# tturturiello/lightweight-snappy

Hardware: AMD Instinct MI355X
Metric: compress + decompress MB/s at 1/2/4/8 MI355X; % HBM roofline; ratio vs ref (higher is better)
Workload: dtype u8

## Files before the change

### lightweight-snappy_amd/csrc/snappy_k2_emit.inc

```
    __shared__ __attribute__((aligned(16))) uint8_t stage_[kK2Stage + 4 + 4 * 64 + 16];
    auto *const stage = (__attribute__((address_space(3))) uint8_t *)stage_;
    const uint32_t lane = threadIdx.x;
    const uint32_t u = blockIdx.x;
    const uint32_t nt = ntok[u];
#if K2_RECORDS
    const uint64_t base = 0;
    const uint32_t L = rec.L;
#else
    const uint64_t base = (uint64_t)u * unit;
    const uint32_t L = (uint32_t)((n - base) < unit ? (n - base) : unit);
#endif
    const uint8_t *src = in + base;
    uint8_t *dst = out + offsets[u];
#if K2_RECORDS
    const uint32_t *tok = rec.tok, *tok_full = rec.tok_full;
#else
    const uint32_t *tok = reinterpret_cast<const uint32_t *>(tokens) + (uint64_t)u * tok_cap;
    const uint32_t *tok_full = reinterpret_cast<const uint32_t *>(tokens) + ((uint64_t)gridDim.x + u) * tok_cap;
#endif
    if (blockIdx.y == 0) {
        if (hdr_mode == SNAPPY_HDR_EVERY_UNIT) varint_put(L, dst, lane);
        else if (hdr_mode == SNAPPY_HDR_FIRST_UNIT && (K2_RECORDS || u == 0)) varint_put(header_value, dst, lane);
    }
    uint32_t kwn[kK2Per];
    auto load_kw = [&](uint32_t c, uint32_t *k) {
#pragma unroll
        for (uint32_t i = 0; i < kK2Per; i++) {
            const uint32_t t = c + kK2Per * lane + i;
            k[i] = tok[t < nt ? t : 0u];
        }
    };
    auto load_se = [&](uint32_t sg) {
#if K2_RECORDS
        return *reinterpret_cast<const uint2 *>(rec.segu + 2 * (sg * kK2Seg <= nt ? sg : 0u));
#else
        return *reinterpret_cast<const uint2 *>(seg_off + 2 * ((uint64_t)u * segs + (sg * kK2Seg <= nt ? sg : 0u)));
#endif
    };
    if (blockIdx.y * kK2Seg <= nt) load_kw(blockIdx.y * kK2Seg, kwn);
    uint2 sen = load_se(blockIdx.y);
    for (uint32_t sg = blockIdx.y; sg * kK2Seg <= nt; sg += gridDim.y) {
    const uint2 se = sen;
    sen = load_se(sg + gridDim.y);
    uint32_t o = se.x, carry = se.y;
    for (uint32_t c = sg * kK2Seg; c < (sg + 1) * kK2Seg && c <= nt; c += kK2Pass) {

    uint32_t gap[kK2Per], len[kK2Per], off[kK2Per], pe[kK2Per], litn[kK2Per], hl[kK2Per], sz[kK2Per];
    bool live[kK2Per];
    uint32_t lspan = 0;
    uint32_t kw[kK2Per];
#pragma unroll
    for (uint32_t i = 0; i < kK2Per; i++) kw[i] = kwn[i];
    {
        uint32_t cn = c + kK2Pass;
        if (!(cn < (sg + 1) * kK2Seg && cn <= nt)) cn = (sg + gridDim.y) * kK2Seg;
        if (cn <= nt) load_kw(cn, kwn);
    }
#pragma unroll
    for (uint32_t i = 0; i < kK2Per; i++) {
        const uint32_t t = c + kK2Per * lane + i;
        const bool has = t < nt;
        live[i] = t <= nt;
        const uint32_t k = has ? kw[i] : 0xFFFFFFFFu;
        const uint32_t lc = (k >> 16) & 0xFF, gc = k >> 24;
        off[i] = has ? k & 0xFFFF : 0u;
        gap[i] = has ? gc : 0u;
        len[i] = has ? lc + 4 : 0u;
        if (has && (lc == 255 || gc == 255)) {
            const uint32_t f = tok_full[t];
            gap[i] = f & 0xFFFF;
            len[i] = f >> 16;
        }
        lspan += gap[i] + len[i];
    }
    uint32_t span_tot;
    uint32_t cur = carry + wave_excl_scan(lspan, lane, &span_tot);
    uint32_t lsum = 0;
#pragma unroll
    for (uint32_t i = 0; i < kK2Per; i++) {
        const uint32_t t = c + kK2Per * lane + i;
        pe[i] = cur;
        litn[i] = t < nt ? gap[i] : (t == nt ? L - cur : 0u);
        cur += gap[i] + len[i];
        hl[i] = litn[i] ? (litn[i] <= 60 ? 1 : (litn[i] <= 256 ? 2 : 3)) : 0;
        sz[i] = hl[i] + litn[i] + ((live[i] && len[i]) ? copy_bytes(len[i], off[i]) : 0);
        lsum += sz[i];
    }
    uint32_t total;
    uint32_t rel = wave_excl_scan(lsum, lane, &total);
    const bool staged = total <= kK2Stage;
    const uint32_t sb = staged ? (uint32_t)(reinterpret_cast<uintptr_t>(dst + o) & 3) : 0u;
    uint64_t longs[kK2Per];
    uint32_t d0v[kK2Per];
    uint32_t lw[kK2Per][5], lsh[kK2Per];
    bool wide[kK2Per];
#pragma unroll
    for (uint32_t i = 0; i < kK2Per; i++) {
        wide[i] = base + pe[i] + 20 <= n;
        const bool ld = !SNAPPY_K2_NOLIT && staged && wide[i] && live[i] && litn[i] != 0 && litn[i] <= 16;
        const uintptr_t sa = reinterpret_cast<uintptr_t>(src + pe[i]);
        lsh[i] = (uint32_t)(sa & 3);
        const auto *aw = reinterpret_cast<const __attribute__((address_space(1))) uint32_t *>(
            ld ? sa - lsh[i] : reinterpret_cast<uintptr_t>(tok));
#pragma unroll
        for (uint32_t j = 0; j < 5; j++) lw[i][j] = aw[j];
    }
#pragma unroll
    for (uint32_t i = 0; i < kK2Per; i++) {
        const bool wide_ok = wide[i];
        if (staged) put_element_lds(stage, rel + sb, src, pe[i], litn[i], hl[i], len[i], off[i], wide_ok, live[i], lane,
                                    lw[i], lsh[i]);
        else if (live[i]) put_element(dst + o + rel, src, pe[i], litn[i], hl[i], len[i], off[i], wide_ok);
        longs[i] = __ballot(live[i] && litn[i] > 16);
        d0v[i] = rel + sb + hl[i];
        rel += sz[i];
    }
#pragma unroll
    for (uint32_t i = 0; i < kK2Per && !SNAPPY_K2_NOLIT; i++) {
        if (staged) k2_long_literals(stage, src, longs[i], litn[i], pe[i], d0v[i], lane);
        else k2_long_literals(dst + o, src, in + n, longs[i], litn[i], pe[i], d0v[i], lane);
    }
    if (staged) {
        __builtin_amdgcn_wave_barrier();
        uint8_t *g = dst + o;
        uint32_t head = (4 - sb) & 3;
        if (head > total) head = total;
        if (lane < head) g[lane] = stage[sb + lane];
        const uint32_t nw = (total - head) >> 2;
        uint32_t *gw = reinterpret_cast<uint32_t *>(g + head);
        const auto *sw = reinterpret_cast<const __attribute__((address_space(3))) uint32_t *>(stage + sb + head);
        for (uint32_t k = lane; k < nw; k += 64) gw[k] = sw[k];
        const uint32_t tail0 = head + 4 * nw;
        if (lane < total - tail0) g[tail0 + lane] = stage[sb + tail0 + lane];
    }
    __builtin_amdgcn_wave_barrier();
    o += total;
    carry += span_tot;
    }
    }
```

### lightweight-snappy_amd/csrc/snappy_kernels.hip

```cpp
#include <hip/hip_runtime.h>
#include <stdint.h>
#include <type_traits>

#include "snappy_kernels.h"

#ifndef SNAPPY_TU
#define SNAPPY_TU 0
#endif
#define SNAPPY_TU_COMPRESS (SNAPPY_TU != 2)
#define SNAPPY_TU_DECODE (SNAPPY_TU != 1)

#if ((defined(SNAPPY_K2_NOLIT) && SNAPPY_K2_NOLIT) || defined(SNAPPY_K4_NOFAR)) && !defined(SNAPPY_MEASUREMENT_BUILD)
#error "SNAPPY_K2_NOLIT / SNAPPY_K4_NOFAR write wrong output: measurement builds only (-DSNAPPY_MEASUREMENT_BUILD)"
#endif

namespace snappy_amd {

__device__ int amdgcn_writelane(int val, int lanesel, int old) __asm("llvm.amdgcn.writelane.i32");


constexpr uint32_t kTable = 4096;
constexpr uint32_t kMul = 0x1e35a7bdu;

typedef uint32_t u32x4 __attribute__((ext_vector_type(4)));
// ... 51 lines not shown
        if constexpr (BIG) _rv = REG_OF_V(_rr & (kRegs - 1));                                       \
        else _rv = REG_OF_V(_rr);                                                                   \
        _rv;                                                                                        \
    })

#define REG_PAIR_V(r, lo, hi)                                                                        \
    do {                                                                                             \
        asm volatile("s_set_gpr_idx_on %[ri], gpr_idx(SRC0)\n\tv_mov_b32 %[olo], v2\n\t"             \
                     "v_mov_b32 %[ohi], v3\n\ts_set_gpr_idx_off"                                     \
                     : [olo] "=&v"(lo), [ohi] "=&v"(hi)                                              \
                     : [ri] "s"((uint32_t)(r)), "{v[2:33]}"(g0), "{v[34:65]}"(g1), "{v[66:97]}"(g2),      \
                       "{v[98:129]}"(g3));                                                           \
    } while (0)
#define REG_PAIR(r, lo, hi)                                                                          \
    do {                                                                                             \
        const uint32_t _pr = (r);                                                                    \
        if constexpr (BIG) {                                  \
            const uint32_t _pq = _pr & (kRegs - 1);                                                  \
            if (__builtin_expect(_pq != kRegs - 1, 1)) REG_PAIR_V(_pq, lo, hi);                      \
            else { lo = REG_OF_V(kRegs - 1); hi = REG_OF_V(0); }                                     \
        } else {                                                                                     \
            REG_PAIR_V(_pr, lo, hi);                                                                 \
        }                                                                                            \
    } while (0)

#define DW_LANES(dd)                                                                                 \
    ({                                                                                               \
        const uint32_t _d = (dd);                                                                    \
        const uint32_t _R = _d >> 6, _l0 = _d & 63;                                                  \
                  \
                      \
        uint32_t _r0, _r1;                                                                           \
        REG_PAIR(_R, _r0, _r1);                                                                      \
        const uint32_t _m = lane >= _l0 ? _r0 : _r1;                                                 \
        (uint32_t)__builtin_amdgcn_ds_bpermute((int)((_d + lane) << 2), (int)_m);    \
    })

__device__ __forceinline__ uint32_t wave_shl1(uint32_t v)
{
    return (uint32_t)__builtin_amdgcn_update_dpp(0, (int)v, 0x130, 0xF, 0xF, true);
}
__device__ __forceinline__ uint32_t wave_shr1(uint32_t v)
{
    return (uint32_t)__builtin_amdgcn_update_dpp(0, (int)v, 0x138, 0xF, 0xF, true);
}

__device__ __forceinline__ uint32_t bytes_at(uint32_t cur, uint32_t next, uint32_t x)
{
    return __builtin_amdgcn_alignbyte(next, cur, x);
}

template <uint32_t D>
__device__ __forceinline__ uint32_t nearest_same_key(uint32_t w)
{
    static_assert(D <= 16, "d << 8 must stay below the key");
    const uint32_t x0 = w & 0xFFFF0000u;
    uint32_t xs = w, best = 0xFFFFFFFFu, k100;
    asm("v_mov_b32 %0, 0x100" : "=v"(k100));
#pragma unroll
    for (uint32_t d = 1; d <= D; d++) {
        xs = wave_shr1(xs) + k100;
        best = __builtin_elementwise_min(best, xs ^ x0);
    }
    return best;
}

__device__ __forceinline__ uint32_t varint_len(uint64_t v)
{
    uint32_t len = 1;
    while (v >= 128) { v >>= 7; len++; }
    return len;
}

__device__ __forceinline__ uint32_t literal_bytes(uint32_t n)
{
    return n + (n <= 60 ? 1 : (n <= 256 ? 2 : 3));
}

__device__ __forceinline__ uint32_t copy_bytes(uint32_t len, uint32_t off)
{
    const uint32_t n64 = len > 68 ? (len - 68 + 63) >> 6 : 0;
    const uint32_t rem = len - 64 * n64;
    const uint32_t has60 = rem > 64 ? 1u : 0u;
    const uint32_t last = has60 ? rem - 60 : rem;
    return 3 * (n64 + has60) + ((last < 12 && off < 2048) ? 2 : 3);
}

__device__ __forceinline__ uint32_t eqm(uint32_t x) { return (uint32_t)((int32_t)(x - 1) >> 31); }

template <int N>
__device__ __forceinline__ uint32_t shz(uint32_t v)
{
    return (uint32_t)__builtin_amdgcn_mov_dpp((int)v, 0x110 + N, 0xF, 0xF, true);
}

template <int N>
__device__ __forceinline__ uint32_t tconf_step(uint32_t h, uint32_t a, uint32_t notdup)
{
    const uint32_t hs = shz<N>(h), as = shz<N>(a);
    if constexpr (N == 1) return eqm(h ^ hs) | eqm(h ^ as) | (eqm(a ^ hs) & notdup);
    else return eqm(h ^ hs) | eqm(h ^ as) | eqm(a ^ hs);
}

template <int W>
__device__ __forceinline__ uint32_t tconf(uint32_t h, uint32_t a, uint32_t notdup)
{
    static_assert(W >= 1 && W <= 4, "W-probe rounds speculate at most 4 probes");
    uint32_t c = 0;
    if constexpr (W > 1) c |= tconf_step<1>(h, a, notdup);
    if constexpr (W > 2) c |= tconf_step<2>(h, a, notdup);
    if constexpr (W > 3) c |= tconf_step<3>(h, a, notdup);
    return c;
}

#ifndef SNAPPY_K1R_DMAX
#define SNAPPY_K1R_DMAX 13
#endif
#ifndef SNAPPY_K1R_DMAX64
#define SNAPPY_K1R_DMAX64 12
#endif
#ifndef SNAPPY_K1R_LSMIN
#define SNAPPY_K1R_LSMIN 4
#endif
#ifndef SNAPPY_K1R_RMIN
#define SNAPPY_K1R_RMIN 2
#endif
#ifndef SNAPPY_K1R_WINDOW
#define SNAPPY_K1R_WINDOW 4
#endif


#if defined(SNAPPY_K1R_LSTAMPS) || defined(SNAPPY_K1R_RSTAMPS)
#define MSTAMP(var)                                                                         \
    do {                                                                                    \
        __builtin_amdgcn_sched_barrier(0);                                                  \
        asm volatile("s_memtime %0\n\ts_waitcnt lgkmcnt(0)" : "=s"(var)::"memory");        \
        __builtin_amdgcn_sched_barrier(0);                                                  \
    } while (0)
#endif
#if defined(SNAPPY_K1R_RSTAMPS)
#define RSTAMP(var) MSTAMP(var)
#else
#define RSTAMP(var) do { } while (0)
#endif
#if defined(SNAPPY_K1R_LSTAMPS)
#define LSTAMP(var) MSTAMP(var)
#define LSEG(i, a, b) seg[i] += (b) - (a)
#else
#define LSTAMP(var) do { } while (0)
#define LSEG(i, a, b) do { } while (0)
#endif

#ifndef SNAPPY_K2_PASS
#define SNAPPY_K2_PASS 128u
#endif
constexpr uint32_t kK2Seg = SNAPPY_K2_SEG;
constexpr uint32_t kK2Pass = SNAPPY_K2_PASS;
[[maybe_unused]] constexpr uint32_t kK2Per = kK2Pass / 64;
static_assert(kK2Pass % 64 == 0 && kK2Seg % kK2Pass == 0, "K2: passes of 64 k tokens dividing a segment");

template <uint32_t CTRL, uint32_t ROWS>
__device__ __forceinline__ uint32_t dpp0(uint32_t x)
{
    return (uint32_t)__builtin_amdgcn_update_dpp(0, (int)x, CTRL, ROWS, 0xF, true);
}

__device__ __forceinline__ uint32_t wave_incl_scan(uint32_t x)
{
    x += dpp0<0x111, 0xF>(x);
    x += dpp0<0x112, 0xF>(x);
    x += dpp0<0x114, 0xF>(x);
    x += dpp0<0x118, 0xF>(x);
    x += dpp0<0x142, 0xA>(x);
    x += dpp0<0x143, 0xC>(x);
    return x;
}

__device__ __forceinline__ uint32_t wave_excl_scan(uint32_t v, uint32_t lane, uint32_t *total)
{
    (void)lane;
    const uint32_t x = wave_incl_scan(v);
    *total = (uint32_t)__builtin_amdgcn_readlane((int)x, 63);
    return x - v;
}


struct K1Record {
    uint32_t u;
    uint32_t L;
    const uint8_t *src;
    uint32_t *tok, *tok_full, *segu;
};

template <bool BIG, bool REC = false>
__device__ __forceinline__ void k1r_body(const uint8_t *__restrict__ in, uint64_t n, uint32_t unit,
                                         uint32_t hdr_mode, uint64_t header_value,
                                         uint2 *__restrict__ tokens, uint32_t tok_cap,
                                         uint32_t *__restrict__ ntok_out, uint32_t *__restrict__ sizes,
                                         uint32_t *__restrict__ seg_off, uint32_t segs, const K1Record rec = {})
{
    constexpr int W = SNAPPY_K1R_WINDOW;
    constexpr uint32_t DMAX = BIG ? SNAPPY_K1R_DMAX64 : SNAPPY_K1R_DMAX;
    static_assert(SNAPPY_K1R_LSMIN >= 4 && SNAPPY_K1R_LSMIN <= 32, "lane-space rounds need skip < 64 - 3");
    static_assert(DMAX >= 2 && DMAX <= 16, "DMAX: 2..16 (kcap <= 15 keeps the lane masks in range)");
    constexpr uint32_t kSlots = kTable + 1;
    constexpr uint32_t kTagBase = 2 * kSlots + 6;
    __shared__ __attribute__((aligned(16))) uint8_t tbl_[kTagBase + kSlots + 7];
    constexpr uint32_t kDummy = 2 * kTable;
    auto *const tbl = (__attribute__((address_space(3))) uint8_t *)tbl_;
#define TBL_READ3(adr)                                                                              \
    ({                                                                                             \
        const uint32_t _a = (adr);                                                                 \
        u16x2 _v;                                                                                  \
        _v.x = *(__attribute__((address_space(3))) uint16_t *)(tbl + _a);                          \
        _v.y = (uint16_t)tbl[(_a >> 1) + kTagBase];                                                \
        __builtin_bit_cast(uint32_t, _v);                                                          \
    })
#define TBL_WRITE3(adr, word)                                                                       \
    do {                                                                                           \
        const uint32_t _a = (adr), _w = (word);                                                    \
        *(__attribute__((address_space(3))) uint16_t *)(tbl + _a) = (uint16_t)_w;                   \
        tbl[(_a >> 1) + kTagBase] = (uint8_t)(_w >> 16);                                           \
    } while (0)
#define TBL_ADR(h) (2 * (h))
#define TBL_READ_ENT(adr)                                                                           \
    do {                                                                                           \
        const uint32_t _a = (adr);                                                                 \
        ent = *(__attribute__((address_space(3))) uint16_t *)(tbl + _a);                           \
        ent_t = tbl[(_a >> 1) + kTagBase];                                                         \
    } while (0)
#define TBL_READ(h) TBL_READ3(2 * (h))
#define TBL_WRITE(s, word) TBL_WRITE3(2 * (s), word)
#define TAG_OF(v) __builtin_amdgcn_ubfe((v) * kMul, shift - 8, 8)
#define TBL_INSERT(cond) TBL_WRITE3((cond) ? adr : kDummy, word)
#define LDS_ORDER() asm volatile("" ::: "memory")
#define TAG_EQ(e, w) ((((e) ^ (w)) & 0xFF0000u) == 0)
    const uint32_t lane = threadIdx.x;
    const uint32_t u = REC ? rec.u : blockIdx.x;
    const uint64_t base = REC ? 0 : (uint64_t)u * unit;
    const uint32_t L = REC ? rec.L : (uint32_t)((n - base) < unit ? (n - base) : unit);
    const uint8_t *src = REC ? rec.src : in + base;
#ifdef SNAPPY_K1R_STATS
    const uint64_t t_start = clock64();
    (void)t_start;
#endif

    v32 g0, g1, g2, g3;
    const bool aligned = ((reinterpret_cast<uintptr_t>(src) & 3) == 0);
    auto load_dw = [&](uint32_t k) -> uint32_t {
        const uint32_t b = 4 * k;
        uint32_t w = 0;
        if (b + 4 <= L && aligned) {
            w = __builtin_nontemporal_load(reinterpret_cast<const uint32_t *>(src + b));
        } else if (b < L) {
            for (uint32_t k = 0; k < 4; k++)
                if (b + k < L) w |= (uint32_t)src[b + k] << (8 * k);
        }
        return w;
    };
    auto load_word = [&](uint32_t i) -> uint32_t { return load_dw(64 * i + lane); };
#pragma unroll
    for (int i = 0; i < (int)kRegs; i++) {
        const uint32_t w = load_word(i);
        if (i < 32) g0[i] = w;
        else if (i < 64) g1[i - 32] = w;
        else if (i < 96) g2[i - 64] = w;
        else g3[i - 96] = w;
    }

    uint32_t seg_hi = kRegs;
#ifdef SNAPPY_K1R_STATS
    uint32_t n_farc = 0, n_reload = 0;
#define K1R_COUNT(x) (x)++
#else
#define K1R_COUNT(x) do { } while (0)
#endif
    __shared__ uint32_t ring_stage[64];
    uint32_t staged = 0;
    auto stage = [&](uint32_t sg) {
        if constexpr (BIG) {
            staged = 0;
            if (aligned && 256 * (sg + 1) <= L) {
                const uint32_t lds = (uint32_t)(uintptr_t)(__attribute__((address_space(3))) uint32_t *)ring_stage;
                uint32_t m0_save, voff;
                asm volatile("s_mov_b32 %0, m0\n\ts_mov_b32 m0, %2\n\tv_lshlrev_b32 %1, 2, %3\n\t"
                             "global_load_lds_dword %1, %4\n\ts_mov_b32 m0, %0"
                             : "=&s"(m0_save), "=&v"(voff)
                             : "s"(lds), "v"(lane), "s"(src + 256 * sg)
                             : "memory");
                staged = sg + 1;
            }
        }
    };
    stage(seg_hi);
    auto ring_to = [&](uint32_t need, auto pf) {
        if constexpr (BIG) {
            if (__builtin_expect(need <= seg_hi, 1)) return;
            uint32_t sg = need - seg_hi > kRegs ? need - kRegs : seg_hi;
            if (decltype(pf)::value && staged == sg + 1) {
                asm volatile("s_waitcnt vmcnt(0)" ::: "memory");
                const uint32_t lds = (uint32_t)(uintptr_t)(__attribute__((address_space(3))) uint32_t *)ring_stage;
                uint32_t w;
                asm volatile("v_lshl_add_u32 %0, %1, 2, %2\n\tds_read_b32 %0, %0\n\ts_waitcnt lgkmcnt(0)"
                             : "=&v"(w) : "v"(lane), "s"(lds) : "memory");
                REG_SET_V(sg & (kRegs - 1), w);
                sg++;
            }
// ... 938 lines not shown

template <bool BIG>
__device__ __forceinline__ void kr1_record(const uint8_t *__restrict__ in, const uint64_t *__restrict__ off_len,
                                           const uint32_t *__restrict__ list, const uint64_t *__restrict__ sbase,
                                           uint32_t *__restrict__ scratch, uint32_t *__restrict__ ntok_out,
                                           uint32_t *__restrict__ sizes)
{
    K1Record rec;
    rec.u = rfl(list[blockIdx.x]);
    rec.L = rfl((uint32_t)off_len[2 * (uint64_t)rec.u + 1]);
    rec.src = in + rfl64(off_len[2 * (uint64_t)rec.u]);
    const uint32_t tok_cap = records_tok_cap(rec.L);
    rec.tok = scratch + rfl64(sbase[rec.u]);
    rec.tok_full = rec.tok + tok_cap;
    rec.segu = rec.tok_full + tok_cap;
    k1r_body<BIG, true>(nullptr, 0, 0, SNAPPY_HDR_EVERY_UNIT, 0, nullptr, 0, ntok_out, sizes, nullptr, 0, rec);
}

#if SNAPPY_TU_COMPRESS
__global__ __launch_bounds__(64, 3) void kr1_match_records(const uint8_t *__restrict__ in,
                                                            const uint64_t *__restrict__ off_len,
                                                            const uint32_t *__restrict__ list,
                                                            const uint64_t *__restrict__ sbase,
                                                            uint32_t *__restrict__ scratch,
                                                            uint32_t *__restrict__ ntok_out,
                                                            uint32_t *__restrict__ sizes)
{
    kr1_record<false>(in, off_len, list, sbase, scratch, ntok_out, sizes);
}

__global__ __launch_bounds__(64, 3) void kr1_match_records64(const uint8_t *__restrict__ in,
                                                              const uint64_t *__restrict__ off_len,
                                                              const uint32_t *__restrict__ list,
                                                              const uint64_t *__restrict__ sbase,
                                                              uint32_t *__restrict__ scratch,
                                                              uint32_t *__restrict__ ntok_out,
                                                              uint32_t *__restrict__ sizes)
{
    kr1_record<true>(in, off_len, list, sbase, scratch, ntok_out, sizes);
}
#endif

template <bool BIG>
__device__ __forceinline__ void kr1_lunit(const uint8_t *__restrict__ in, const uint64_t *__restrict__ off_len,
                                          const uint32_t *__restrict__ list, const uint32_t *__restrict__ urec,
                                          const uint64_t *__restrict__ ubase, const uint64_t *__restrict__ sbase,
                                          uint32_t *__restrict__ scratch, uint32_t *__restrict__ ntok_out,
                                          uint32_t *__restrict__ sizes)
{
    K1Record rec;
    rec.u = rfl(list[blockIdx.x]);
    const uint32_t r = rfl(urec[rec.u]);
    const uint32_t blk = rec.u - rfl((uint32_t)ubase[r]);
    const uint64_t len = rfl64(off_len[2 * (uint64_t)r + 1]);
    const uint64_t at = (uint64_t)blk * SNAPPY_BLOCK;
    rec.L = (uint32_t)(len - at < SNAPPY_BLOCK ? len - at : SNAPPY_BLOCK);
    rec.src = in + rfl64(off_len[2 * (uint64_t)r]) + at;
    const uint32_t tok_cap = records_tok_cap(rec.L);
    rec.tok = scratch + rfl64(sbase[rec.u]);
    rec.tok_full = rec.tok + tok_cap;
    rec.segu = rec.tok_full + tok_cap;
    k1r_body<BIG, true>(nullptr, 0, 0, blk == 0 ? SNAPPY_HDR_FIRST_UNIT : SNAPPY_HDR_NONE, len, nullptr, 0, ntok_out,
                        sizes, nullptr, 0, rec);
}

#if SNAPPY_TU_COMPRESS
__global__ __launch_bounds__(64, 3) void kr1_match_lunits(const uint8_t *__restrict__ in,
                                                           const uint64_t *__restrict__ off_len,
                                                           const uint32_t *__restrict__ list,
                                                           const uint32_t *__restrict__ urec,
                                                           const uint64_t *__restrict__ ubase,
                                                           const uint64_t *__restrict__ sbase,
                                                           uint32_t *__restrict__ scratch,
                                                           uint32_t *__restrict__ ntok_out,
                                                           uint32_t *__restrict__ sizes)
{
    kr1_lunit<false>(in, off_len, list, urec, ubase, sbase, scratch, ntok_out, sizes);
}

__global__ __launch_bounds__(64, 3) void kr1_match_lunits64(const uint8_t *__restrict__ in,
                                                             const uint64_t *__restrict__ off_len,
                                                             const uint32_t *__restrict__ list,
                                                             const uint32_t *__restrict__ urec,
                                                             const uint64_t *__restrict__ ubase,
                                                             const uint64_t *__restrict__ sbase,
                                                             uint32_t *__restrict__ scratch,
                                                             uint32_t *__restrict__ ntok_out,
                                                             uint32_t *__restrict__ sizes)
{
    kr1_lunit<true>(in, off_len, list, urec, ubase, sbase, scratch, ntok_out, sizes);
}
#endif

__device__ __forceinline__ uint32_t wave_excl_scan32(uint32_t v, uint32_t *total)
{
    uint32_t x = v;
    x += dpp0<0x111, 0xF>(x);
    x += dpp0<0x112, 0xF>(x);
    x += dpp0<0x114, 0xF>(x);
    x += dpp0<0x118, 0xF>(x);
    x += dpp0<0x142, 0xA>(x);
    *total = (uint32_t)__builtin_amdgcn_readlane((int)x, 31);
    return x - v;
}

template <typename P>
__device__ __forceinline__ void put_copy(P *o, uint32_t len, uint32_t off)
{
    while (len > 68) {
        o[0] = 0xFE; o[1] = (uint8_t)off; o[2] = (uint8_t)(off >> 8);
        o += 3; len -= 64;
    }
    if (len > 64) {
        o[0] = 0xEE; o[1] = (uint8_t)off; o[2] = (uint8_t)(off >> 8);
        o += 3; len -= 60;
    }
    if (len < 12 && off < 2048) {
        o[0] = (uint8_t)((((off >> 8) << 5) + ((len - 4) << 2) + 1));
        o[1] = (uint8_t)off;
    } else {
        o[0] = (uint8_t)(((len - 1) << 2) | 2); o[1] = (uint8_t)off; o[2] = (uint8_t)(off >> 8);
    }
}

template <typename P>
__device__ __forceinline__ void put_element(P *w, const uint8_t *__restrict__ src, uint32_t s0, uint32_t litn,
                                            uint32_t hl, uint32_t len, uint32_t off, bool wide_ok)
{
    if (hl == 1) w[0] = (uint8_t)((litn - 1) << 2);
    else if (hl == 2) { w[0] = 60 << 2; w[1] = (uint8_t)(litn - 1); }
    else if (hl == 3) { w[0] = 61 << 2; w[1] = (uint8_t)(litn - 1); w[2] = (uint8_t)((litn - 1) >> 8); }
    if (litn <= 16) {
        if (wide_ok) {
            const uintptr_t sa = reinterpret_cast<uintptr_t>(src + s0);
            const uint32_t sh = (uint32_t)(sa & 3);
            const uint32_t *aw = reinterpret_cast<const uint32_t *>(sa - sh);
            const uint32_t d0 = aw[0], d1 = aw[1], d2 = aw[2], d3 = aw[3], d4 = aw[4];
            const uint32_t r[4] = {__builtin_amdgcn_alignbyte(d1, d0, sh), __builtin_amdgcn_alignbyte(d2, d1, sh),
                                   __builtin_amdgcn_alignbyte(d3, d2, sh), __builtin_amdgcn_alignbyte(d4, d3, sh)};
#pragma unroll
            for (uint32_t j = 0; j < 16; j++)
                if (j < litn) w[hl + j] = (uint8_t)(r[j >> 2] >> (8 * (j & 3)));
        } else {
            for (uint32_t j = 0; j < litn; j++) w[hl + j] = src[s0 + j];
        }
    }
    if (len) put_copy(w + hl + litn, len, off);
}

#ifndef SNAPPY_K2_STAGE
#define SNAPPY_K2_STAGE 4096
#endif
constexpr uint32_t kK2Stage = SNAPPY_K2_STAGE;

__device__ __forceinline__ void put_element_lds(__attribute__((address_space(3))) uint8_t *stage, uint32_t at,
                                                const uint8_t *__restrict__ src, uint32_t s0, uint32_t litn,
                                                uint32_t hl, uint32_t len, uint32_t off, bool wide_ok, bool live,
                                                uint32_t lane, const uint32_t *lw, uint32_t sh)
{
    const uint32_t dum = kK2Stage + 4 + 4 * lane;
#define K2_ST8(cond, adr, v) stage[(cond) ? (adr) : dum] = (uint8_t)(v)
    const uint32_t lm1 = litn - 1;
    K2_ST8(live && hl >= 1, at, hl == 1 ? lm1 << 2 : (hl == 2 ? 60u << 2 : 61u << 2));
    K2_ST8(live && hl >= 2, at + 1, lm1);
    K2_ST8(live && hl == 3, at + 2, lm1 >> 8);
    const uint32_t lp = at + hl;
    if (litn <= 16) {
        if (wide_ok) {
            const uint32_t r0 = __builtin_amdgcn_alignbyte(lw[1], lw[0], sh), r1 = __builtin_amdgcn_alignbyte(lw[2], lw[1], sh);
            const uint32_t r2 = __builtin_amdgcn_alignbyte(lw[3], lw[2], sh), r3 = __builtin_amdgcn_alignbyte(lw[4], lw[3], sh);
#define K2_ST32(k, r) *(__attribute__((address_space(3))) u32u *)(stage + (live && 4 * (k) + 4 <= litn ? lp + 4 * (k) : dum)) = (r)
            K2_ST32(0, r0); K2_ST32(1, r1); K2_ST32(2, r2); K2_ST32(3, r3);
#undef K2_ST32
            const uint32_t fb = litn & ~3u, rem = litn & 3u;
            const uint32_t rt = fb == 0 ? r0 : (fb == 4 ? r1 : (fb == 8 ? r2 : r3));
            K2_ST8(live && rem > 0, lp + fb, rt);
            K2_ST8(live && rem > 1, lp + fb + 1, rt >> 8);
            K2_ST8(live && rem > 2, lp + fb + 2, rt >> 16);
        } else if (live) {
            for (uint32_t j = 0; j < litn; j++) stage[lp + j] = src[s0 + j];
        }
    }
    const uint32_t cp = lp + litn;
    if (len <= 64) {
        const bool c1 = len < 12 && off < 2048;
        const bool has = live && len != 0;
        K2_ST8(has, cp, c1 ? (((off >> 8) << 5) + ((len - 4) << 2) + 1) : (((len - 1) << 2) | 2));
        K2_ST8(has, cp + 1, off);
        K2_ST8(has && !c1, cp + 2, off >> 8);
    } else if (live) {
        put_copy(stage + cp, len, off);
    }
#undef K2_ST8
}

__device__ __forceinline__ void k2_long_literals(__attribute__((address_space(3))) uint8_t *w,
                                                 const uint8_t *__restrict__ src, uint64_t longs, uint32_t litn,
                                                 uint32_t s0v, uint32_t d0v, uint32_t lane)
{
    while (longs) {
        const uint32_t k = (uint32_t)__builtin_ctzll(longs);
        longs &= longs - 1;
        const uint32_t ln = __builtin_amdgcn_readlane(litn, k);
        const uint32_t s0 = __builtin_amdgcn_readlane(s0v, k);
        const uint32_t d0 = __builtin_amdgcn_readlane(d0v, k);
        for (uint32_t j0 = 0; j0 < ln; j0 += 512) {
            uint8_t v[8];
#pragma unroll
            for (uint32_t q = 0; q < 8; q++) {
                const uint32_t j = j0 + 64 * q + lane;
                v[q] = j < ln ? src[s0 + j] : 0;
            }
#pragma unroll
            for (uint32_t q = 0; q < 8; q++) {
                const uint32_t j = j0 + 64 * q + lane;
                if (j < ln) w[d0 + j] = v[q];
            }
        }
    }
}

__device__ __forceinline__ void k2_long_literals(uint8_t *w, const uint8_t *__restrict__ src,
                                                 const uint8_t *__restrict__ end, uint64_t longs, uint32_t litn,
                                                 uint32_t s0v, uint32_t d0v, uint32_t lane)
{
    while (longs) {
        const uint32_t k = (uint32_t)__builtin_ctzll(longs);
        longs &= longs - 1;
        const uint32_t ln = __builtin_amdgcn_readlane(litn, k);
        const uint8_t *s = src + __builtin_amdgcn_readlane(s0v, k);
        uint8_t *d = w + __builtin_amdgcn_readlane(d0v, k);
        uint32_t head = (uint32_t)((4 - (reinterpret_cast<uintptr_t>(d) & 3)) & 3);
        if (head > ln) head = ln;
        if (lane < head) d[lane] = s[lane];
        const uint32_t nw = (ln - head) >> 2;
        const uint8_t *sb = s + head;
        const uint32_t sh = (uint32_t)(reinterpret_cast<uintptr_t>(sb) & 3);
        const uint32_t *sa = reinterpret_cast<const uint32_t *>(sb - sh);
        uint32_t *dw = reinterpret_cast<uint32_t *>(d + head);
        for (uint32_t k0 = 0; k0 < nw; k0 += 256) {
            uint32_t lo[4], hi[4];
#pragma unroll
            for (uint32_t q = 0; q < 4; q++) {
                const uint32_t kk = k0 + 64 * q + lane;
                lo[q] = hi[q] = 0;
                if (kk < nw) {
                    lo[q] = sa[kk];
                    if (sh) {
                        const uint8_t *pb = reinterpret_cast<const uint8_t *>(sa + kk + 1);
                        if (pb + 4 <= end) hi[q] = sa[kk + 1];
                        else for (uint32_t t = 0; t < sh; t++) hi[q] |= (uint32_t)pb[t] << (8 * t);
                    }
                }
            }
#pragma unroll
            for (uint32_t q = 0; q < 4; q++) {
                const uint32_t kk = k0 + 64 * q + lane;
                if (kk < nw) dw[kk] = __builtin_amdgcn_alignbyte(hi[q], lo[q], sh);
            }
        }
        const uint32_t t0 = head + 4 * nw;
        if (lane < ln - t0) d[t0 + lane] = s[t0 + lane];
    }
}

#ifndef SNAPPY_K2_NOLIT
#define SNAPPY_K2_NOLIT 0
#endif
struct K2Record {
    uint32_t L;
    const uint32_t *tok, *tok_full, *segu;
};

#if SNAPPY_TU_COMPRESS
__global__ __launch_bounds__(64, 6) void k2_emit_units(const uint8_t *__restrict__ in, uint64_t n, uint32_t unit,
                                                    uint32_t hdr_mode, uint64_t header_value,
                                                    const uint2 *__restrict__ tokens, uint32_t tok_cap,
                                                    const uint32_t *__restrict__ ntok,
                                                    const uint32_t *__restrict__ seg_off, uint32_t segs,
                                                    const uint64_t *__restrict__ offsets, uint8_t *__restrict__ out)
{
#define K2_RECORDS 0
#include "snappy_k2_emit.inc"
#undef K2_RECORDS
}

__device__ __forceinline__ void kr2_emit_one(const uint8_t *in, const K2Record rec, const uint32_t *ntok,
                                             const uint64_t *offsets, uint8_t *out,
                                             const uint32_t hdr_mode = SNAPPY_HDR_EVERY_UNIT,
                                             const uint64_t header_value = 0)
{
    const uint64_t n = rec.L;
#define K2_RECORDS 1
#include "snappy_k2_emit.inc"
#undef K2_RECORDS
}

__global__ __launch_bounds__(64, 6) void kr2_emit_records(const uint8_t *__restrict__ base,
                                                          const uint64_t *__restrict__ off_len,
                                                          const int32_t *__restrict__ status,
                                                          const uint64_t *__restrict__ sbase,
                                                          const uint32_t *__restrict__ scratch,
                                                          const uint32_t *__restrict__ ntok,
                                                          const uint64_t *__restrict__ offsets,
                                                          uint8_t *__restrict__ out)
{
    const uint32_t r = blockIdx.x;
    const int32_t st = status[r];
    const uint64_t off = off_len[2 * (uint64_t)r], len = off_len[2 * (uint64_t)r + 1], sb = sbase[r];
    if (st < 0) return;
    K2Record rec;
    rec.L = rfl((uint32_t)len);
    if (rec.L == 0) {
        if (blockIdx.y == 0 && threadIdx.x == 0) out[offsets[r]] = 0;
        return;
    }
    const uint32_t tok_cap = records_tok_cap(rec.L);
    rec.tok = scratch + rfl64(sb);
    rec.tok_full = rec.tok + tok_cap;
    rec.segu = rec.tok_full + tok_cap;
    kr2_emit_one(base + rfl64(off), rec, ntok, offsets, out);
}

__global__ __launch_bounds__(64, 6) void kr2_emit_lunits(const uint8_t *__restrict__ base,
                                                         const uint64_t *__restrict__ off_len,
                                                         const uint32_t *__restrict__ urec,
                                                         const uint64_t *__restrict__ ubase,
                                                         const uint64_t *__restrict__ sbase,
                                                         const uint32_t *__restrict__ scratch,
                                                         const uint32_t *__restrict__ ntok,
                                                         const uint64_t *__restrict__ offsets,
                                                         uint8_t *__restrict__ out)
{
    const uint32_t u = blockIdx.x;
    const uint32_t r = rfl(urec[u]);
    const uint64_t sb = sbase[u];
    const uint64_t off = off_len[2 * (uint64_t)r], len = rfl64(off_len[2 * (uint64_t)r + 1]);
    const uint32_t blk = u - rfl((uint32_t)ubase[r]);
    if (len == 0) {
        if (blockIdx.y == 0 && threadIdx.x == 0) out[offsets[u]] = 0;
        return;
    }
    const uint64_t at = (uint64_t)blk * SNAPPY_BLOCK;
    K2Record rec;
    rec.L = (uint32_t)(len - at < SNAPPY_BLOCK ? len - at : SNAPPY_BLOCK);
    const uint32_t tok_cap = records_tok_cap(rec.L);
    rec.tok = scratch + rfl64(sb);
    rec.tok_full = rec.tok + tok_cap;
    rec.segu = rec.tok_full + tok_cap;
    kr2_emit_one(base + rfl64(off) + at, rec, ntok, offsets, out, blk == 0 ? SNAPPY_HDR_FIRST_UNIT : SNAPPY_HDR_NONE,
                 len);
}
#endif

constexpr uint32_t kScanPer = 8;
[[maybe_unused]] constexpr uint32_t kScanTile = 1024 * kScanPer;

#if SNAPPY_TU_COMPRESS
__global__ __launch_bounds__(1024) void k3_scan(const uint32_t *__restrict__ sizes, uint64_t count,
                                                uint64_t *__restrict__ offsets, uint64_t *__restrict__ total)
{
    __shared__ uint32_t tile[kScanTile + kScanTile / 32];
    __shared__ uint32_t wtot[16];
    const uint32_t t = threadIdx.x, lane = t & 63, w = t >> 6;
#define K3_AT(i) ((i) + ((i) >> 5))
    uint64_t carry = 0;
    for (uint64_t b = 0; b < count; b += kScanTile) {
        const uint32_t m = (uint32_t)(count - b < kScanTile ? count - b : kScanTile);
        for (uint32_t i = t; i < kScanTile; i += 1024) tile[K3_AT(i)] = i < m ? sizes[b + i] : 0u;
        __syncthreads();
        uint32_t v[kScanPer], s = 0;
#pragma unroll
        for (uint32_t k = 0; k < kScanPer; k++) {
            v[k] = tile[K3_AT(t * kScanPer + k)];
            s += v[k];
        }
        const uint32_t x = wave_incl_scan(s);
        if (lane == 63) wtot[w] = x;
        __syncthreads();
        if (w == 0) {
            const uint32_t y = lane < 16 ? wtot[lane] : 0u;
            const uint32_t z = wave_incl_scan(y);
            if (lane < 16) wtot[lane] = z - y;
        }
        __syncthreads();
        uint32_t run = wtot[w] + x - s;
#pragma unroll
        for (uint32_t k = 0; k < kScanPer; k++) {
            tile[K3_AT(t * kScanPer + k)] = run;
            run += v[k];
        }
        __syncthreads();
        for (uint32_t i = t; i < m; i += 1024) offsets[b + i] = carry + tile[K3_AT(i)];
        if (t == 1023) wtot[0] = run;
        __syncthreads();
        carry += wtot[0];
        __syncthreads();
    }
#undef K3_AT
    if (t == 0) {
        offsets[count] = carry;
        *total = carry;
    }
}

__global__ __launch_bounds__(64) void k3_scan_wave(const uint32_t *__restrict__ sizes, uint64_t count,
                                                  uint64_t *__restrict__ offsets, uint64_t *__restrict__ total)
{
    const uint32_t lane = threadIdx.x;
    uint64_t carry = 0;
    for (uint64_t b = 0; b < count; b += 64 * kScanPer) {
        uint32_t v[kScanPer], s = 0;
#pragma unroll
        for (uint32_t k = 0; k < kScanPer; k++) {
            const uint64_t i = b + kScanPer * lane + k;
            v[k] = i < count ? sizes[i] : 0u;
            s += v[k];
        }
        uint32_t tot;
        uint32_t run = wave_excl_scan(s, lane, &tot);
#pragma unroll
        for (uint32_t k = 0; k < kScanPer; k++) {
            const uint64_t i = b + kScanPer * lane + k;
            if (i < count) offsets[i] = carry + run;
            run += v[k];
        }
        carry += tot;
    }
    if (lane == 0) {
        offsets[count] = carry;
        *total = carry;
    }
}
#endif

constexpr uint64_t kIdxOffMask = (1ull << 40) - 1;
constexpr uint32_t kIdxSkipShift = 40;
constexpr int32_t kK4Tail = 3;

__device__ __forceinline__ uint32_t load_dw_guarded(const uint8_t *comp, uint64_t a, uint64_t lim)
{
    if (a + 4 <= lim) return __builtin_nontemporal_load(reinterpret_cast<const uint32_t *>(comp + a));
    uint32_t w = 0;
    for (uint32_t k = 0; k < 4; k++)
        if (a + k < lim) w |= (uint32_t)comp[a + k] << (8 * k);
    return w;
}

__device__ __forceinline__ uint32_t load_seg(const uint8_t *comp, uint64_t a0, uint64_t lim, uint32_t lane)
{
    if (a0 + 256 <= lim) return __builtin_nontemporal_load(reinterpret_cast<const uint32_t *>(comp + a0) + lane);
    return load_dw_guarded(comp, a0 + 4 * lane, lim);
}

__device__ __forceinline__ void k4_flush(const uint8_t *ob, uint32_t M, uint8_t *dst, uint32_t F, uint32_t T,
                                         uint32_t lane)
{
    if (T <= F) return;
    if ((reinterpret_cast<uintptr_t>(dst) & 15) == 0) {
        uint32_t a = (F + 15) & ~15u;
        if (a > T) a = T;
        if (F + lane < a) dst[F + lane] = ob[(F + lane) & M];
        const uint32_t e = T & ~15u;
#pragma unroll 1
        for (uint32_t x = a + 16 * lane; x < e; x += 1024)
            *reinterpret_cast<u32x4 *>(dst + x) = *reinterpret_cast<const u32x4 *>(ob + (x & M));
        const uint32_t t0 = e > a ? e : a;
        if (t0 + lane < T) dst[t0 + lane] = ob[(t0 + lane) & M];
    } else {
#pragma unroll 1
        for (uint32_t x = F + lane; x < T; x += 64) dst[x] = ob[x & M];
    }
}

#define K4_LIT_ATTR __noinline__
__device__ K4_LIT_ATTR void k4_literal_hbm(const uint8_t *lsrc, uint32_t kl, uint32_t kop, uint8_t *ob, uint32_t M,
                                               uint8_t *dst, uint32_t lane)
// ... 1569 lines not shown
```

Baseline: 80680.

## Pack emit scans, prefetch long-literal heads, halve pass size, raise occupancy

Computes literal headers and element sizes before the prefix scan, so the span and size scans can be packed into one 32-bit wave scan whenever both fit in 16 bits. The tail literal is patched in afterwards with a readlane. Long literals in the staged path now have their first 128 bytes loaded in groups before put_element_lds and stored afterwards, overlapping those global loads with the element writes. Pass size drops from 128 to 64 tokens and the emit kernels' launch bounds rise from 6 to 8 waves, trading more register pressure and extra per-pass overhead for more occupancy and latency hiding.

```diff
diff --git a/lightweight-snappy_amd/csrc/snappy_k2_emit.inc b/lightweight-snappy_amd/csrc/snappy_k2_emit.inc
--- a/lightweight-snappy_amd/csrc/snappy_k2_emit.inc
+++ b/lightweight-snappy_amd/csrc/snappy_k2_emit.inc
@@ -48,6 +48,7 @@
     uint32_t gap[kK2Per], len[kK2Per], off[kK2Per], pe[kK2Per], litn[kK2Per], hl[kK2Per], sz[kK2Per];
     bool live[kK2Per];
     uint32_t lspan = 0;
+    uint32_t lsum = 0;
     uint32_t kw[kK2Per];
 #pragma unroll
     for (uint32_t i = 0; i < kK2Per; i++) kw[i] = kwn[i];
@@ -72,22 +73,36 @@
             len[i] = f >> 16;
         }
         lspan += gap[i] + len[i];
+        litn[i] = gap[i];
+        hl[i] = literal_header(litn[i]);
+        sz[i] = hl[i] + litn[i] + (len[i] ? copy_bytes(len[i], off[i]) : 0);
+        lsum += sz[i];
     }
-    uint32_t span_tot;
-    uint32_t cur = carry + wave_excl_scan(lspan, lane, &span_tot);
-    uint32_t lsum = 0;
+    uint32_t span_tot, total, cur, rel;
+    if (__ballot((lspan | lsum) > kK2Packed) == 0) {
+        uint32_t pt;
+        const uint32_t px = wave_excl_scan(lspan | lsum << 16, lane, &pt);
+        cur = carry + (px & 0xFFFF);
+        rel = px >> 16;
+        span_tot = pt & 0xFFFF;
+        total = pt >> 16;
+    } else {
+        cur = carry + wave_excl_scan(lspan, lane, &span_tot);
+        rel = wave_excl_scan(lsum, lane, &total);
+    }
+    uint32_t tsz = 0;
 #pragma unroll
     for (uint32_t i = 0; i < kK2Per; i++) {
         const uint32_t t = c + kK2Per * lane + i;
         pe[i] = cur;
-        litn[i] = t < nt ? gap[i] : (t == nt ? L - cur : 0u);
+        if (t == nt) {
+            litn[i] = L - cur;
+            hl[i] = literal_header(litn[i]);
+            tsz = sz[i] = hl[i] + litn[i];
+        }
         cur += gap[i] + len[i];
-        hl[i] = litn[i] ? (litn[i] <= 60 ? 1 : (litn[i] <= 256 ? 2 : 3)) : 0;
-        sz[i] = hl[i] + litn[i] + ((live[i] && len[i]) ? copy_bytes(len[i], off[i]) : 0);
-        lsum += sz[i];
     }
-    uint32_t total;
-    uint32_t rel = wave_excl_scan(lsum, lane, &total);
+    if (nt - c < kK2Pass) total += (uint32_t)__builtin_amdgcn_readlane((int)tsz, (nt - c) / kK2Per);
     const bool staged = total <= kK2Stage;
     const uint32_t sb = staged ? (uint32_t)(reinterpret_cast<uintptr_t>(dst + o) & 3) : 0u;
     uint64_t longs[kK2Per];
@@ -108,18 +123,36 @@
 #pragma unroll
     for (uint32_t i = 0; i < kK2Per; i++) {
         const bool wide_ok = wide[i];
-        if (staged) put_element_lds(stage, rel + sb, src, pe[i], litn[i], hl[i], len[i], off[i], wide_ok, live[i], lane,
-                                    lw[i], lsh[i]);
-        else if (live[i]) put_element(dst + o + rel, src, pe[i], litn[i], hl[i], len[i], off[i], wide_ok);
-        longs[i] = __ballot(live[i] && litn[i] > 16);
+        longs[i] = SNAPPY_K2_NOLIT ? 0 : __ballot(live[i] && litn[i] > 16);
         d0v[i] = rel + sb + hl[i];
+        if (staged) {
+            K2Longs lg;
+            uint64_t more = longs[i];
+            bool have = more != 0;
+            if (have) more = k2_longs_load(lg, src, more, litn[i], pe[i], d0v[i], lane);
+            put_element_lds(stage, rel + sb, src, pe[i], litn[i], hl[i], len[i], off[i], wide_ok, live[i], lane,
+                            lw[i], lsh[i]);
+            while (have) {
+                k2_longs_store(stage, lg, lane);
+                have = more != 0;
+                if (have) more = k2_longs_load(lg, src, more, litn[i], pe[i], d0v[i], lane);
+            }
+            if (longs[i])
+                k2_long_literals(stage, src, __ballot(live[i] && litn[i] > kK2LongHead), litn[i], pe[i], d0v[i], lane,
+                                 kK2LongHead);
+        } else if (live[i]) {
+            put_element(dst + o + rel, src, pe[i], litn[i], hl[i], len[i], off[i], wide_ok);
+        }
         rel += sz[i];
     }
+    if (!staged) {
 #pragma unroll
-    for (uint32_t i = 0; i < kK2Per && !SNAPPY_K2_NOLIT; i++) {
-        if (staged) k2_long_literals(stage, src, longs[i], litn[i], pe[i], d0v[i], lane);
-        else k2_long_literals(dst + o, src, in + n, longs[i], litn[i], pe[i], d0v[i], lane);
+        for (uint32_t i = 0; i < kK2Per; i++)
+            k2_long_literals(dst + o, src, in + n, longs[i], litn[i], pe[i], d0v[i], lane);
     }
+#pragma unroll
+    for (uint32_t i = 0; i < kK2Per; i++)
+        asm volatile("" ::"v"(kwn[i]), "v"(lw[i][0]), "v"(lw[i][1]), "v"(lw[i][2]), "v"(lw[i][3]), "v"(lw[i][4]));
     if (staged) {
         __builtin_amdgcn_wave_barrier();
         uint8_t *g = dst + o;
diff --git a/lightweight-snappy_amd/csrc/snappy_kernels.hip b/lightweight-snappy_amd/csrc/snappy_kernels.hip
--- a/lightweight-snappy_amd/csrc/snappy_kernels.hip
+++ b/lightweight-snappy_amd/csrc/snappy_kernels.hip
@@ -227,7 +227,7 @@
 #endif
 
 #ifndef SNAPPY_K2_PASS
-#define SNAPPY_K2_PASS 128u
+#define SNAPPY_K2_PASS 64u
 #endif
 constexpr uint32_t kK2Seg = SNAPPY_K2_SEG;
 constexpr uint32_t kK2Pass = SNAPPY_K2_PASS;
@@ -1472,6 +1472,12 @@
 #define SNAPPY_K2_STAGE 4096
 #endif
 constexpr uint32_t kK2Stage = SNAPPY_K2_STAGE;
+[[maybe_unused]] constexpr uint32_t kK2Packed = 1021;
+
+__device__ __forceinline__ uint32_t literal_header(uint32_t litn)
+{
+    return litn ? (litn <= 60 ? 1 : (litn <= 256 ? 2 : 3)) : 0;
+}
 
 __device__ __forceinline__ void put_element_lds(__attribute__((address_space(3))) uint8_t *stage, uint32_t at,
                                                 const uint8_t *__restrict__ src, uint32_t s0, uint32_t litn,
@@ -1514,9 +1520,51 @@
 #undef K2_ST8
 }
 
+constexpr uint32_t kK2LongGroup = 4, kK2LongHead = 128;
+struct K2Longs {
+    uint32_t ln[kK2LongGroup], s0[kK2LongGroup], d0[kK2LongGroup];
+    uint8_t v[kK2LongGroup][kK2LongHead / 64];
+};
+
+__device__ __forceinline__ uint64_t k2_longs_load(K2Longs &g, const uint8_t *__restrict__ src, uint64_t longs,
+                                                  uint32_t litn, uint32_t s0v, uint32_t d0v, uint32_t lane)
+{
+    uint32_t k = 0;
+#pragma unroll
+    for (uint32_t q = 0; q < kK2LongGroup; q++) {
+        if (longs) {
+            k = (uint32_t)__builtin_ctzll(longs);
+            longs &= longs - 1;
+        }
+        g.ln[q] = __builtin_amdgcn_readlane(litn, k);
+        g.s0[q] = __builtin_amdgcn_readlane(s0v, k);
+        g.d0[q] = __builtin_amdgcn_readlane(d0v, k);
+#pragma unroll
+        for (uint32_t h = 0; h < kK2LongHead / 64; h++) {
+            const uint32_t j = 64 * h + lane;
+            g.v[q][h] = src[g.s0[q] + (j < g.ln[q] ? j : g.ln[q] - 1)];
+        }
+    }
+    return longs;
+}
+
+__device__ __forceinline__ void k2_longs_store(__attribute__((address_space(3))) uint8_t *w, const K2Longs &g,
+                                               uint32_t lane)
+{
+    const uint32_t dum = kK2Stage + 4 + 4 * lane;
+#pragma unroll
+    for (uint32_t q = 0; q < kK2LongGroup; q++) {
+#pragma unroll
+        for (uint32_t h = 0; h < kK2LongHead / 64; h++) {
+            const uint32_t j = 64 * h + lane;
+            w[j < g.ln[q] ? g.d0[q] + j : dum] = g.v[q][h];
+        }
+    }
+}
+
 __device__ __forceinline__ void k2_long_literals(__attribute__((address_space(3))) uint8_t *w,
                                                  const uint8_t *__restrict__ src, uint64_t longs, uint32_t litn,
-                                                 uint32_t s0v, uint32_t d0v, uint32_t lane)
+                                                 uint32_t s0v, uint32_t d0v, uint32_t lane, uint32_t from)
 {
     while (longs) {
         const uint32_t k = (uint32_t)__builtin_ctzll(longs);
@@ -1524,7 +1572,7 @@
         const uint32_t ln = __builtin_amdgcn_readlane(litn, k);
         const uint32_t s0 = __builtin_amdgcn_readlane(s0v, k);
         const uint32_t d0 = __builtin_amdgcn_readlane(d0v, k);
-        for (uint32_t j0 = 0; j0 < ln; j0 += 512) {
+        for (uint32_t j0 = from; j0 < ln; j0 += 512) {
             uint8_t v[8];
 #pragma unroll
             for (uint32_t q = 0; q < 8; q++) {
@@ -1593,7 +1641,7 @@
 };
 
 #if SNAPPY_TU_COMPRESS
-__global__ __launch_bounds__(64, 6) void k2_emit_units(const uint8_t *__restrict__ in, uint64_t n, uint32_t unit,
+__global__ __launch_bounds__(64, 8) void k2_emit_units(const uint8_t *__restrict__ in, uint64_t n, uint32_t unit,
                                                     uint32_t hdr_mode, uint64_t header_value,
                                                     const uint2 *__restrict__ tokens, uint32_t tok_cap,
                                                     const uint32_t *__restrict__ ntok,
@@ -1616,7 +1664,7 @@
 #undef K2_RECORDS
 }
 
-__global__ __launch_bounds__(64, 6) void kr2_emit_records(const uint8_t *__restrict__ base,
+__global__ __launch_bounds__(64, 8) void kr2_emit_records(const uint8_t *__restrict__ base,
                                                           const uint64_t *__restrict__ off_len,
                                                           const int32_t *__restrict__ status,
                                                           const uint64_t *__restrict__ sbase,
@@ -1642,7 +1690,7 @@
     kr2_emit_one(base + rfl64(off), rec, ntok, offsets, out);
 }
 
-__global__ __launch_bounds__(64, 6) void kr2_emit_lunits(const uint8_t *__restrict__ base,
+__global__ __launch_bounds__(64, 8) void kr2_emit_lunits(const uint8_t *__restrict__ base,
                                                          const uint64_t *__restrict__ off_len,
                                                          const uint32_t *__restrict__ urec,
                                                          const uint64_t *__restrict__ ubase,
```

After: 80700 (median of 5 runs). About the same (+0.0%).
